# LemonATsu/UNet-PhaseGen

Measured on NVIDIA B200. Metric: audio_seconds_per_second_mag_to_phase_to_wave, higher is better.
Workload: dtype f16x3/f16x2/f16-fp32acc (two-product fp16 on d1,u2; single fp16 product = TF32 operand rounding on u1)

## Files before the change

unet-phasegen_b200/csrc/stft.cu:

```cuda
#include "common.cuh"
#include "stft_core.cuh"

namespace pg {
using namespace pgfft;

constexpr int kStftThreads = 256;

template <int NC> struct FrameCfg {
    static constexpr int TG = NC / 16;
    static constexpr int FC = kStftThreads / TG;
    static constexpr int NFFT = 2 * NC;
    static constexpr int HOP = NFFT / 4;
    static constexpr int PL = padded_len2(NC);
    static constexpr size_t smem_stft() { return sizeof(float2) * (Radix<NC, false>::TOTAL + NC + (size_t)FC * PL); }
    static constexpr int RING = FC + 3;
    static constexpr size_t smem_istft() { return sizeof(float2) * (Radix<NC, true>::TOTAL + NC + (size_t)RING * PL + NC ) + sizeof(float) * HOP; }
};

template <int TG> struct FrameSync {
    int slot;
    __device__ __forceinline__ void operator()() const {
        if (TG <= 32) __syncwarp();
        else asm volatile("bar.sync %0, %1;" ::"r"(slot + 1), "r"(TG) : "memory");
    }
};

__device__ __forceinline__ float fast_log1p_mag(float re, float im) {
    const float m2 = fmaf(re, re, im * im);
    float mag, l2;
    asm("sqrt.approx.ftz.f32 %0, %1;" : "=f"(mag) : "f"(m2));
    asm("lg2.approx.ftz.f32 %0, %1;" : "=f"(l2) : "f"(1.0f + mag));
    return l2 * 0.693147180559945f;
}

template <int NC, int FAST, bool RAGGED>
__global__ void __launch_bounds__(kStftThreads, 3)
stft_kernel(const float* __restrict__ wave, int N, int T, const float2* __restrict__ tw_g, int mode,
            float* __restrict__ out_a, float* __restrict__ out_b,
            uint16_t* __restrict__ op_hi, uint16_t* __restrict__ op_lo,
            long long op_batch_stride, int op_fmt, int frames_per_cta, const float* __restrict__ proj_mag,
            float std_mean, float std_inv, const int* __restrict__ clip_samples, const int* __restrict__ clip_frames) {
    using Cfg = FrameCfg<NC>;
    using R = Radix<NC, false>;
    extern __shared__ float2 smem2[];
    cpx* tabs = reinterpret_cast<cpx*>(smem2);
    cpx* win = tabs + R::TOTAL;
    cpx* bufs = win + NC;

    const int tid = threadIdx.x;
    const cpx* twc = reinterpret_cast<const cpx*>(tw_g);
    for (int e = tid; e < R::TOTAL; e += kStftThreads) tabs[e] = table_entry<NC, false>(twc, e);
    for (int m = tid; m < NC; m += kStftThreads)
        win[m] = {0.25f - 0.25f * tw_g[2 * m].x, 0.25f - 0.25f * tw_g[2 * m + 1].x};
    __syncthreads();

    const int b = blockIdx.y;
    const int n_b = RAGGED ? min(__ldg(clip_samples + b), N) : N;
    const int T_b = RAGGED ? min(__ldg(clip_frames + b), T) : T;
    const int N_b = RAGGED ? (T_b - 1) * Cfg::HOP : N;
    const int slot = tid / Cfg::TG, t = tid % Cfg::TG;
    cpx* s = bufs + slot * Cfg::PL;
    const FrameSync<Cfg::TG> sync{slot};
    const float* w = wave + (size_t)b * N;
    const bool aligned = (N & 1) == 0 && (reinterpret_cast<uintptr_t>(wave) & 7) == 0;
    const int f_begin = blockIdx.x * frames_per_cta;

    for (int f0 = f_begin; f0 < f_begin + frames_per_cta && f0 < T; f0 += Cfg::FC) {
        const int frame = f0 + slot;
        const bool live = frame < T;
        const int p0 = frame * Cfg::HOP - NC;
        cpx v[16];
        if (live && aligned && p0 >= 0 && p0 + Cfg::NFFT <= n_b) {
#pragma unroll
            for (int r = 0; r < 16; ++r) {
                const int m = t + r * Cfg::TG;
                const float2 xv = __ldg(reinterpret_cast<const float2*>(w + p0) + m);
                const cpx wv = win[m];
                v[r] = {xv.x * wv.x, xv.y * wv.y};
            }
        } else if (live && (!RAGGED || frame < T_b)) {
#pragma unroll
            for (int r = 0; r < 16; ++r) {
                const int m = t + r * Cfg::TG;
                int n0 = p0 + 2 * m, n1 = n0 + 1;
                if (n0 < 0) n0 = -n0;
                if (n0 >= N_b) n0 = 2 * (N_b - 1) - n0;
                if (n1 < 0) n1 = -n1;
                if (n1 >= N_b) n1 = 2 * (N_b - 1) - n1;
                const float x0 = (n0 >= 0 && n0 < n_b) ? __ldg(w + n0) : 0.f;
                const float x1 = (n1 >= 0 && n1 < n_b) ? __ldg(w + n1) : 0.f;
                const cpx wv = win[m];
                v[r] = {x0 * wv.x, x1 * wv.y};
            }
        } else {
#pragma unroll
            for (int r = 0; r < 16; ++r) v[r] = {0.f, 0.f};
        }
        fwd_phase0<NC>(s, t, v);
        sync();
        fwd_phase1<NC>(s, t, tabs, sync);
        sync();

        const size_t row = ((size_t)b * T + frame) * NC;
        const size_t orow = (size_t)b * op_batch_stride + (size_t)frame * NC;
        auto emit = [&](int bin, cpx x) {
            if (FAST) {
                const float a = fast_log1p_mag(x.x, x.y);
                uint16_t hi, lo;
                split16(a, FAST == 2 ? PG_FMT_F16 : PG_FMT_BF16, hi, lo);
                out_a[row + bin - 1] = a;
                op_hi[orow + bin - 1] = hi;
                op_lo[orow + bin - 1] = lo;
                return;
            }
            if (bin == NC) x.y = 0.f;
            float a, ph = 0.f;
            if (mode == PG_STFT_PROJECT) {
                const float m2 = fmaf(x.x, x.x, x.y * x.y);
                const float inv = m2 > 0.f ? rsqrtf(m2) : 0.f;
                const float g = __ldg(proj_mag + row + bin - 1);
                a = m2 > 0.f ? g * x.x * inv : g;
                ph = g * x.y * inv;
            } else if (mode == PG_STFT_LOGMAG || mode == PG_STFT_PAIRS) {
                if (mode == PG_STFT_PAIRS) {
                    x.x = (x.x - std_mean) * std_inv;
                    x.y = (x.y - std_mean) * std_inv;
                }
                a = fast_log1p_mag(x.x, x.y);
                if (out_b) ph = atan2f(x.y, x.x);
            } else {
                a = x.x; ph = x.y;
            }
            if (out_a) out_a[row + bin - 1] = a;
            if (out_b) out_b[row + bin - 1] = ph;
            if (op_hi) {
                uint16_t hi, lo;
                split16(a, op_fmt, hi, lo);
                op_hi[orow + bin - 1] = hi;
                if (op_lo) op_lo[orow + bin - 1] = lo;
            }
        };
        if (NC == 512) {
            if (live) fwd_fused_last_512(s, t, tabs, emit);
        } else {
            fwd_phase2_unfused<NC>(s, t, tabs, sync);
            sync();
            if (live) fwd_post_generic<NC>(s, t, tabs, emit);
        }
        sync();
    }
}

__device__ __forceinline__ cpx spec_value(float a, float p, int mode) {
    if (mode == PG_SPEC_CARTESIAN) return {a, p};
    float mag = a;
    if (mode == PG_SPEC_POLAR_LOG) mag = __expf(a) - 1.0f;
    return {mag * __cosf(p), mag * __sinf(p)};
}

template <int NC, bool FAST, bool RAGGED>
__global__ void __launch_bounds__(kStftThreads)
istft_kernel(const float* __restrict__ in_a, const float* __restrict__ in_b, int mode, int T,
             const float2* __restrict__ tw_g, float* __restrict__ wave,
             unsigned* __restrict__ peak_bits, int* __restrict__ nonfinite, int blocks_per_cta,
             const float2* __restrict__ b_ss, int b_ss_stride, const int* __restrict__ clip_frames,
             const int* __restrict__ clip_samples) {
    using Cfg = FrameCfg<NC>;
    using R = Radix<NC, true>;
    constexpr int FC = Cfg::FC, HOP = Cfg::HOP;
    extern __shared__ float2 smem2[];
    float* wss_full = reinterpret_cast<float*>(smem2);
    cpx* tabs = reinterpret_cast<cpx*>(wss_full + HOP);
    cpx* win = tabs + R::TOTAL;
    cpx* ring = win + NC;
    float2* ss_tab = reinterpret_cast<float2*>(ring + (size_t)Cfg::RING * Cfg::PL);

    const int tid = threadIdx.x;
    const cpx* twc = reinterpret_cast<const cpx*>(tw_g);
    for (int e = tid; e < R::TOTAL; e += kStftThreads) tabs[e] = table_entry<NC, true>(twc, e);
    for (int m = tid; m < NC; m += kStftThreads) win[m] = {0.5f - 0.5f * tw_g[2 * m].x, 0.5f - 0.5f * tw_g[2 * m + 1].x};
    for (int i = tid; i < HOP; i += kStftThreads) {
        float acc = 0.f;
#pragma unroll
        for (int q = 0; q < 4; ++q) { const float wn = 0.5f - 0.5f * tw_g[q * HOP + i].x; acc += wn * wn; }
        wss_full[i] = acc > 1.17549435e-38f ? 1.0f / acc : 1.0f;
    }
    const int b = blockIdx.y;
    const int T_b = RAGGED ? min(__ldg(clip_frames + b), T) : T;
    const int n_b = RAGGED ? __ldg(clip_samples + b) : 0;
    if (b_ss) for (int m = tid; m < NC; m += kStftThreads) ss_tab[m] = __ldg(b_ss + (size_t)b * b_ss_stride + m);
    __syncthreads();

    const int J0 = blockIdx.x * blocks_per_cta;
    const int J1 = min(J0 + blocks_per_cta, T - 1);
    const int F0 = J0 - 1;
    const int n_iter = (J1 - J0 + 3 + FC - 1) / FC;
    const int slot = tid / Cfg::TG, t = tid % Cfg::TG;
    const FrameSync<Cfg::TG> sync{slot};
    const float scale = 0.5f / NC;
    float* wv = wave + (size_t)b * (size_t)(T - 1) * HOP;
    float pk = 0.f;
    bool bad = false;

    float ra[16], rb[16];
    auto is_live = [&](int frame) { return frame >= 0 && frame < T_b && frame <= J1 + 1; };
    auto fetch = [&](int frame) {
        if (!is_live(frame)) return;
        const size_t row = ((size_t)b * T + frame) * NC;
#pragma unroll
        for (int j = 0; j < 16; ++j) {
            const size_t idx = row + inv_bin<NC>(t, j) - 1;
            ra[j] = __ldg(in_a + idx);
            rb[j] = (FAST || in_b) ? __ldg(in_b + idx) : 0.f;
        }
    };
    fetch(F0 + slot);

    for (int it = 0; it < n_iter; ++it) {
        const int F = F0 + it * FC;
        const int frame = F + slot;
        const bool live = is_live(frame);
        cpx* s = ring + (size_t)((frame - F0) % Cfg::RING) * Cfg::PL;
        if (live) {
            cpx x[16];
#pragma unroll
            for (int j = 0; j < 16; ++j) {
                float pb = rb[j];
                if (b_ss) { const float2 ss = ss_tab[inv_bin<NC>(t, j) - 1]; pb = fmaf(pb, ss.x, ss.y); }
                x[j] = spec_value(ra[j], pb, FAST ? (int)PG_SPEC_POLAR_LOG : mode);
            }
            if (NC == 512) inv_fused_first_512(s, t, tabs, scale, x);
            else inv_pre_generic<NC>(s, t, tabs, scale, x);
        }
        if (it + 1 < n_iter) fetch(frame + FC);
        sync();
        inv_passes<NC>(s, t, tabs, win, sync);
        __syncthreads();

        const int lo = max(J0, F - 2), hi = min(J1, F + FC - 2);
        for (int u = tid; u < (hi - lo) * (HOP / 4); u += kStftThreads) {
            const int jb = lo + u / (HOP / 4), i = (u % (HOP / 4)) * 4;
            float4 acc = make_float4(0.f, 0.f, 0.f, 0.f), wss;
            const bool interior = jb >= 1 && jb + 2 < T_b;
            if (interior) wss = *reinterpret_cast<const float4*>(wss_full + i);
            else wss = make_float4(0.f, 0.f, 0.f, 0.f);
#pragma unroll
            for (int q = 0; q < 4; ++q) {
                const int fr = jb - 1 + q;
                if (fr < 0 || fr >= T_b) continue;
                const cpx* fb = ring + (size_t)((fr - F0) % Cfg::RING) * Cfg::PL;
                const int m = ((3 - q) * HOP + i) >> 1;
                const cpx z0 = fb[pad2(m)], z1 = fb[pad2(m + 1)];
                acc.x += z0.x; acc.y += z0.y; acc.z += z1.x; acc.w += z1.y;
                if (!interior) {
                    const cpx w0 = win[m], w1 = win[m + 1];
                    wss.x += w0.x * w0.x; wss.y += w0.y * w0.y; wss.z += w1.x * w1.x; wss.w += w1.y * w1.y;
                }
            }
            if (!interior) {
                wss.x = wss.x > 1.17549435e-38f ? 1.0f / wss.x : 1.0f; wss.y = wss.y > 1.17549435e-38f ? 1.0f / wss.y : 1.0f;
                wss.z = wss.z > 1.17549435e-38f ? 1.0f / wss.z : 1.0f; wss.w = wss.w > 1.17549435e-38f ? 1.0f / wss.w : 1.0f;
            }
            float4 y;
            y.x = acc.x * wss.x; y.y = acc.y * wss.y; y.z = acc.z * wss.z; y.w = acc.w * wss.w;
            if (RAGGED && jb >= T_b - 1) y = make_float4(0.f, 0.f, 0.f, 0.f);
            const float mx = fmaxf(fmaxf(fabsf(y.x), fabsf(y.y)), fmaxf(fabsf(y.z), fabsf(y.w)));
            if (!(mx <= 3.402823466e+38f) || y.x != y.x || y.y != y.y || y.z != y.z || y.w != y.w) bad = true;
            pk = fmaxf(pk, mx);
            if (RAGGED) {
                const int n = jb * HOP + i;
                if (n >= n_b) y.x = 0.f;
                if (n + 1 >= n_b) y.y = 0.f;
                if (n + 2 >= n_b) y.z = 0.f;
                if (n + 3 >= n_b) y.w = 0.f;
            }
            *reinterpret_cast<float4*>(wv + (size_t)jb * HOP + i) = y;
        }
        __syncthreads();
    }
    if (peak_bits) {
#pragma unroll
        for (int o = 16; o; o >>= 1) pk = fmaxf(pk, __shfl_xor_sync(0xffffffffu, pk, o));
        if ((tid & 31) == 0 && pk > 0.f) atomicMax(peak_bits + b, __float_as_uint(pk));
    }
    if (nonfinite && bad) atomicOr(nonfinite + b, 1);
}

__global__ void peak_normalize_kernel(float* __restrict__ wave, const unsigned* __restrict__ peak_bits, int n) {
    const int b = blockIdx.y;
    float pk = __uint_as_float(peak_bits[b]);
    if (!(pk >= 1.17549435e-38f)) return;
    float inv = 1.0f / pk;
    float* w = wave + (size_t)b * n;
    if ((n & 3) == 0) {
        float4* w4 = reinterpret_cast<float4*>(w);
        for (int i = blockIdx.x * blockDim.x + threadIdx.x; i < n / 4; i += gridDim.x * blockDim.x) {
            float4 v = w4[i];
            v.x *= inv; v.y *= inv; v.z *= inv; v.w *= inv;
            w4[i] = v;
        }
    } else {
        for (int i = blockIdx.x * blockDim.x + threadIdx.x; i < n; i += gridDim.x * blockDim.x) w[i] = w[i] * inv;
    }
}

__global__ void __launch_bounds__(256)
stitch_kernel(const float* __restrict__ windows, int n_windows, int win, int step, int world, int per_rank,
              float* __restrict__ out, long long n_out, unsigned* __restrict__ peak_bits) {
    const int ov = win - step;
    const float inv_ov = ov > 0 ? 1.0f / (float)ov : 0.f;
    float pk = 0.f;
    for (long long n = (long long)blockIdx.x * blockDim.x + threadIdx.x; n < n_out; n += (long long)gridDim.x * blockDim.x) {
        long long i1 = n / step; if (i1 > n_windows - 1) i1 = n_windows - 1;
        float acc = 0.f;
#pragma unroll
        for (int q = 0; q < 2; ++q) {
            const long long i = i1 - q;
            if (i < 0) continue;
            const long long o = n - i * step;
            if (o >= win) continue;
            float g = 1.f;
            if (i > 0 && o < ov) g = 0.5f - 0.5f * cospif((float)o * inv_ov);
            else if (i < n_windows - 1 && o >= win - ov) g = 0.5f + 0.5f * cospif((float)(o - (win - ov)) * inv_ov);
            const size_t slot = (size_t)(i % world) * per_rank + (size_t)(i / world);
            acc = fmaf(__ldg(windows + slot * win + o), g, acc);
        }
        out[n] = acc;
        pk = fmaxf(pk, fabsf(acc));
    }
    if (peak_bits) {
#pragma unroll
        for (int o = 16; o; o >>= 1) pk = fmaxf(pk, __shfl_xor_sync(0xffffffffu, pk, o));
        if ((threadIdx.x & 31) == 0 && pk > 0.f) atomicMax(peak_bits, __float_as_uint(pk));
    }
}

template <int NC, bool RAGGED>
static auto stft_variant(bool fast, int fmt) {
    return !fast ? stft_kernel<NC, 0, RAGGED> : fmt == PG_FMT_F16 ? stft_kernel<NC, 2, RAGGED> : stft_kernel<NC, 1, RAGGED>;
}

template <int NC>
static int launch_stft(const float* wave, int B, int N, int T, const float* tw, int mode, float* a, float* bq,
                       uint16_t* hi, uint16_t* lo, long long bs, int fmt, cudaStream_t st, const float* proj_mag = nullptr,
                       float std_mean = 0.f, float std_inv = 1.f, const int* clip_samples = nullptr, const int* clip_frames = nullptr) {
    using Cfg = FrameCfg<NC>;
    const bool fast = mode == PG_STFT_LOGMAG && a && !bq && hi && lo;
    auto k = clip_samples ? stft_variant<NC, true>(fast, fmt) : stft_variant<NC, false>(fast, fmt);
    const size_t sm = Cfg::smem_stft();
    static bool configured_dev[kMaxDevices] = {};
    bool& configured = configured_dev[current_device_slot()];
    if (!configured) {
        for (int f = 0; f < 3; ++f)
            for (auto kv : {stft_variant<NC, false>(f > 0, f == 2 ? PG_FMT_F16 : PG_FMT_BF16),
                            stft_variant<NC, true>(f > 0, f == 2 ? PG_FMT_F16 : PG_FMT_BF16)})
                cudaFuncSetAttribute(kv, cudaFuncAttributeMaxDynamicSharedMemorySize, (int)sm);
        configured = true;
    }
    const int frames_per_cta = Cfg::FC * 4;
    dim3 grid((T + frames_per_cta - 1) / frames_per_cta, B);
    k<<<grid, kStftThreads, sm, st>>>(wave, N, T, reinterpret_cast<const float2*>(tw), mode, a, bq, hi, lo, bs, fmt, frames_per_cta, proj_mag,
                                      std_mean, std_inv, clip_samples, clip_frames);
    return check_launch("stft_kernel");
}

template <int NC>
static int launch_istft(const float* a, const float* bq, int mode, int B, int T, const float* tw, float* wave,
                        float* peak, int* nonfinite, cudaStream_t st, const float* b_ss, int b_ss_stride,
                        const int* clip_frames = nullptr, const int* clip_samples = nullptr) {
    using Cfg = FrameCfg<NC>;
    const bool fast = mode == PG_SPEC_POLAR_LOG && bq;
    auto k = clip_frames ? (fast ? istft_kernel<NC, true, true> : istft_kernel<NC, false, true>)
                         : (fast ? istft_kernel<NC, true, false> : istft_kernel<NC, false, false>);
    const size_t sm = Cfg::smem_istft();
    static bool configured_dev[kMaxDevices] = {};
    bool& configured = configured_dev[current_device_slot()];
    if (!configured) {
        for (auto kv : {istft_kernel<NC, true, false>, istft_kernel<NC, false, false>, istft_kernel<NC, true, true>, istft_kernel<NC, false, true>})
            cudaFuncSetAttribute(kv, cudaFuncAttributeMaxDynamicSharedMemorySize, (int)sm);
        configured = true;
    }
    const int blocks_per_cta = 11 * Cfg::FC - 3;
    dim3 grid((T - 1 + blocks_per_cta - 1) / blocks_per_cta, B);
    k<<<grid, kStftThreads, sm, st>>>(a, bq, mode, T, reinterpret_cast<const float2*>(tw), wave,
                                     reinterpret_cast<unsigned*>(peak), nonfinite, blocks_per_cta,
                                     reinterpret_cast<const float2*>(b_ss), b_ss_stride, clip_frames, clip_samples);
    return check_launch("istft_kernel");
}

}

extern "C" int pg_stft_num_frames(int n_samples, int hop) { return hop > 0 ? 1 + n_samples / hop : 0; }

static int stft_entry(const float* wave, int B, int N, int n_fft, int hop, const float* twiddle, int mode,
                      float* out_a, float* out_b, uint16_t* op_hi, uint16_t* op_lo,
                      int64_t op_batch_stride, int op_fmt, const int* cs, const int* cf, pg_stream stream) {
    PG_REQUIRE(wave && twiddle && B > 0 && N > 0, "pg_stft: null pointer or empty batch");
    PG_REQUIRE(hop * 4 == n_fft, "pg_stft: hop must be n_fft/4 (got n_fft=%d hop=%d)", n_fft, hop);
    PG_REQUIRE(N > n_fft / 2, "pg_stft: reflect padding needs more than n_fft/2 samples (N=%d)", N);
    PG_REQUIRE(mode == PG_STFT_LOGMAG || mode == PG_STFT_REIM, "pg_stft: bad mode %d", mode);
    PG_REQUIRE(B <= 65535, "pg_stft: batch too large for one launch");
    const int T = 1 + N / hop;
    cudaStream_t st = reinterpret_cast<cudaStream_t>(stream);
    switch (n_fft) {
        case 256:  return pg::launch_stft<128>(wave, B, N, T, twiddle, mode, out_a, out_b, op_hi, op_lo, op_batch_stride, op_fmt, st, nullptr, 0.f, 1.f, cs, cf);
        case 512:  return pg::launch_stft<256>(wave, B, N, T, twiddle, mode, out_a, out_b, op_hi, op_lo, op_batch_stride, op_fmt, st, nullptr, 0.f, 1.f, cs, cf);
        case 1024: return pg::launch_stft<512>(wave, B, N, T, twiddle, mode, out_a, out_b, op_hi, op_lo, op_batch_stride, op_fmt, st, nullptr, 0.f, 1.f, cs, cf);
        case 2048: return pg::launch_stft<1024>(wave, B, N, T, twiddle, mode, out_a, out_b, op_hi, op_lo, op_batch_stride, op_fmt, st, nullptr, 0.f, 1.f, cs, cf);
    }
    pg::set_error("pg_stft: n_fft must be 256, 512, 1024 or 2048 (got %d)", n_fft);
    return PG_ERR_UNSUPPORTED;
}

extern "C" int pg_stft(const float* wave, int B, int N, int n_fft, int hop, const float* twiddle, int mode,
                       float* out_a, float* out_b, uint16_t* op_hi, uint16_t* op_lo,
                       int64_t op_batch_stride, int op_fmt, pg_stream stream) {
    return stft_entry(wave, B, N, n_fft, hop, twiddle, mode, out_a, out_b, op_hi, op_lo, op_batch_stride, op_fmt, nullptr, nullptr, stream);
}

extern "C" int pg_stft_ragged(const float* wave, int B, int N, int n_fft, int hop, const float* twiddle, int mode,
                              float* out_a, float* out_b, uint16_t* op_hi, uint16_t* op_lo,
                              int64_t op_batch_stride, int op_fmt, const int* clip_samples, const int* clip_frames, pg_stream stream) {
    PG_REQUIRE(clip_samples && clip_frames, "pg_stft_ragged: null per-clip table");
    if (mode != PG_STFT_LOGMAG) {
        pg::set_error("pg_stft_ragged: only PG_STFT_LOGMAG takes per-clip lengths (got mode %d)", mode);
        return PG_ERR_UNSUPPORTED;
    }
    return stft_entry(wave, B, N, n_fft, hop, twiddle, mode, out_a, out_b, op_hi, op_lo, op_batch_stride, op_fmt, clip_samples, clip_frames, stream);
}

extern "C" int pg_stft_project(const float* wave, int B, int N, int n_fft, int hop, const float* twiddle, const float* mag,
                               float* out_re, float* out_im, pg_stream stream) {
    PG_REQUIRE(wave && twiddle && mag && out_re && out_im && B > 0 && N > 0, "pg_stft_project: null pointer or empty batch");
    PG_REQUIRE(hop * 4 == n_fft, "pg_stft_project: hop must be n_fft/4 (got n_fft=%d hop=%d)", n_fft, hop);
    PG_REQUIRE(N > n_fft / 2, "pg_stft_project: reflect padding needs more than n_fft/2 samples (N=%d)", N);
    PG_REQUIRE(B <= 65535, "pg_stft_project: batch too large for one launch");
    const int T = 1 + N / hop;
    cudaStream_t st = reinterpret_cast<cudaStream_t>(stream);
    switch (n_fft) {
        case 256:  return pg::launch_stft<128>(wave, B, N, T, twiddle, PG_STFT_PROJECT, out_re, out_im, nullptr, nullptr, 0, 0, st, mag);
        case 512:  return pg::launch_stft<256>(wave, B, N, T, twiddle, PG_STFT_PROJECT, out_re, out_im, nullptr, nullptr, 0, 0, st, mag);
        case 1024: return pg::launch_stft<512>(wave, B, N, T, twiddle, PG_STFT_PROJECT, out_re, out_im, nullptr, nullptr, 0, 0, st, mag);
        case 2048: return pg::launch_stft<1024>(wave, B, N, T, twiddle, PG_STFT_PROJECT, out_re, out_im, nullptr, nullptr, 0, 0, st, mag);
    }
    pg::set_error("pg_stft_project: n_fft must be 256, 512, 1024 or 2048 (got %d)", n_fft);
    return PG_ERR_UNSUPPORTED;
}

extern "C" int pg_stft_pairs(const float* wave, int B, int N, int n_fft, int hop, const float* twiddle, float mean, float std,
                             float* out_logmag, float* out_phase, pg_stream stream) {
    PG_REQUIRE(wave && twiddle && out_logmag && out_phase && B > 0 && N > 0, "pg_stft_pairs: null pointer or empty batch");
    PG_REQUIRE(hop * 4 == n_fft, "pg_stft_pairs: hop must be n_fft/4 (got n_fft=%d hop=%d)", n_fft, hop);
    PG_REQUIRE(N > n_fft / 2, "pg_stft_pairs: reflect padding needs more than n_fft/2 samples (N=%d)", N);
    PG_REQUIRE(std > 0.f && B <= 65535, "pg_stft_pairs: std must be positive and B <= 65535");
    const int T = 1 + N / hop;
    cudaStream_t st = reinterpret_cast<cudaStream_t>(stream);
    const float inv = 1.0f / std;
    switch (n_fft) {
        case 256:  return pg::launch_stft<128>(wave, B, N, T, twiddle, PG_STFT_PAIRS, out_logmag, out_phase, nullptr, nullptr, 0, 0, st, nullptr, mean, inv);
        case 512:  return pg::launch_stft<256>(wave, B, N, T, twiddle, PG_STFT_PAIRS, out_logmag, out_phase, nullptr, nullptr, 0, 0, st, nullptr, mean, inv);
        case 1024: return pg::launch_stft<512>(wave, B, N, T, twiddle, PG_STFT_PAIRS, out_logmag, out_phase, nullptr, nullptr, 0, 0, st, nullptr, mean, inv);
        case 2048: return pg::launch_stft<1024>(wave, B, N, T, twiddle, PG_STFT_PAIRS, out_logmag, out_phase, nullptr, nullptr, 0, 0, st, nullptr, mean, inv);
    }
    pg::set_error("pg_stft_pairs: n_fft must be 256, 512, 1024 or 2048 (got %d)", n_fft);
    return PG_ERR_UNSUPPORTED;
}

static int istft_entry(const float* in_a, const float* in_b, int mode, int B, int T, int n_fft, int hop,
                       const float* twiddle, float* wave, float* peak, int* nonfinite,
                       const float* b_scale_shift, int b_ss_per_clip, const int* cf, const int* cs, pg_stream stream) {
    PG_REQUIRE(in_a && twiddle && wave && B > 0 && T > 1, "pg_istft: null pointer or empty input");
    PG_REQUIRE(hop * 4 == n_fft, "pg_istft: hop must be n_fft/4 (got n_fft=%d hop=%d)", n_fft, hop);
    PG_REQUIRE(mode >= PG_SPEC_POLAR_LOG && mode <= PG_SPEC_POLAR_MAG, "pg_istft: bad mode %d", mode);
    PG_REQUIRE(in_b || mode != PG_SPEC_CARTESIAN, "pg_istft: second plane missing");
    PG_REQUIRE(B <= 65535, "pg_istft: batch too large for one launch");
    PG_REQUIRE(!b_scale_shift || in_b, "pg_istft: scale/shift given without a second plane");
    const int ss_stride = b_ss_per_clip ? n_fft / 2 : 0;
    cudaStream_t st = reinterpret_cast<cudaStream_t>(stream);
    if (peak) cudaMemsetAsync(peak, 0, sizeof(float) * B, st);
    if (nonfinite) cudaMemsetAsync(nonfinite, 0, sizeof(int) * B, st);
    switch (n_fft) {
        case 256:  return pg::launch_istft<128>(in_a, in_b, mode, B, T, twiddle, wave, peak, nonfinite, st, b_scale_shift, ss_stride, cf, cs);
        case 512:  return pg::launch_istft<256>(in_a, in_b, mode, B, T, twiddle, wave, peak, nonfinite, st, b_scale_shift, ss_stride, cf, cs);
        case 1024: return pg::launch_istft<512>(in_a, in_b, mode, B, T, twiddle, wave, peak, nonfinite, st, b_scale_shift, ss_stride, cf, cs);
        case 2048: return pg::launch_istft<1024>(in_a, in_b, mode, B, T, twiddle, wave, peak, nonfinite, st, b_scale_shift, ss_stride, cf, cs);
    }
    pg::set_error("pg_istft: n_fft must be 256, 512, 1024 or 2048 (got %d)", n_fft);
    return PG_ERR_UNSUPPORTED;
}

extern "C" int pg_istft(const float* in_a, const float* in_b, int mode, int B, int T, int n_fft, int hop,
                        const float* twiddle, float* wave, float* peak, int* nonfinite,
                        const float* b_scale_shift, int b_ss_per_clip, pg_stream stream) {
    return istft_entry(in_a, in_b, mode, B, T, n_fft, hop, twiddle, wave, peak, nonfinite, b_scale_shift, b_ss_per_clip, nullptr, nullptr, stream);
}

extern "C" int pg_istft_ragged(const float* in_a, const float* in_b, int mode, int B, int T, int n_fft, int hop,
                               const float* twiddle, float* wave, float* peak, int* nonfinite,
                               const float* b_scale_shift, int b_ss_per_clip, const int* clip_frames, const int* clip_samples,
                               pg_stream stream) {
    PG_REQUIRE(clip_frames && clip_samples, "pg_istft_ragged: null per-clip table");
    return istft_entry(in_a, in_b, mode, B, T, n_fft, hop, twiddle, wave, peak, nonfinite, b_scale_shift, b_ss_per_clip, clip_frames, clip_samples, stream);
}

extern "C" int pg_peak_normalize(float* wave, const float* peak, int B, int N, pg_stream stream) {
    PG_REQUIRE(wave && peak && B > 0 && N > 0 && B <= 65535, "pg_peak_normalize: bad arguments");
    dim3 grid((N + 1023) / 1024 < 64 ? (N + 1023) / 1024 : 64, B);
    pg::peak_normalize_kernel<<<grid, 256, 0, reinterpret_cast<cudaStream_t>(stream)>>>(
        wave, reinterpret_cast<const unsigned*>(peak), N);
    return pg::check_launch("peak_normalize_kernel");
}

extern "C" int pg_stitch(const float* windows, int n_windows, int win, int step, int world, int per_rank, float* out,
                         int64_t n_out, float* peak, pg_stream stream) {
    PG_REQUIRE(windows && out && n_windows > 0 && win > 0 && n_out > 0, "pg_stitch: bad arguments");
    PG_REQUIRE(step > 0 && step <= win && 2 * step >= win, "pg_stitch: step must lie in [win/2, win] (got win=%d step=%d)", win, step);
    PG_REQUIRE(world >= 1 && per_rank >= (n_windows + world - 1) / world, "pg_stitch: per_rank too small for %d windows on %d ranks", n_windows, world);
    PG_REQUIRE(n_out <= (int64_t)win + (int64_t)(n_windows - 1) * step, "pg_stitch: n_out exceeds the span of the windows");
    cudaStream_t st = reinterpret_cast<cudaStream_t>(stream);
    if (peak) cudaMemsetAsync(peak, 0, sizeof(float), st);
    long long blocks = (n_out + 255) / 256; if (blocks > 148 * 16) blocks = 148 * 16;
    pg::stitch_kernel<<<(int)blocks, 256, 0, st>>>(windows, n_windows, win, step, world, per_rank, out, n_out, reinterpret_cast<unsigned*>(peak));
    return pg::check_launch("stitch_kernel");
}
```

unet-phasegen_b200/phasegen/ops.py:

```python
import ctypes as C
import math

import torch

from . import _lib
from ._lib import (ActDst, ConvDesc, ConvEpilogue, PG_EPI_ACT, PG_EPI_NORM_ACT, PG_EPI_RAW, PG_CONV, PG_CONV_TRANSPOSE, PG_DT_BF16, PG_DT_BF16_SPLIT, PG_DT_F16,
                   PG_DT_F16_SPLIT, PG_DT_F32, PG_DT_NONE, PG_FMT_BF16, PG_FMT_F16, PG_PREC_BF16, PG_PREC_BF16X3,
                   PG_PREC_F16X2, PG_PREC_F16X3, PG_PREC_FP32_SIMT, PG_SPEC_CARTESIAN, PG_SPEC_POLAR_LOG,
                   PG_SPEC_POLAR_MAG, PG_STFT_LOGMAG, PG_STFT_REIM)

SUPPORTED_N_FFT = (256, 512, 1024, 2048)


def _stream(t=None):
    dev = t.device if isinstance(t, torch.Tensor) and t.is_cuda else None
    return C.c_void_p(torch.cuda.current_stream(dev).cuda_stream)


def _ptr(t):
    return C.c_void_p(t.data_ptr()) if t is not None else C.c_void_p(0)


def _fmt(t):
    if t is None or t.dtype == torch.bfloat16:
        return PG_FMT_BF16
    if t.dtype == torch.float16:
        return PG_FMT_F16
    raise RuntimeError(f"phasegen: operand planes must be bfloat16 or float16, got {t.dtype}")


def _need_cuda(t, name, dtype=torch.float32):
    if not isinstance(t, torch.Tensor) or not t.is_cuda:
        raise RuntimeError(f"phasegen: `{name}` must be a CUDA tensor (there is no CPU path)")
    if t.dtype != dtype:
        raise RuntimeError(f"phasegen: `{name}` must be {dtype}, got {t.dtype}")
    if t.device.index != torch.cuda.current_device():
        raise RuntimeError(f"phasegen: `{name}` lives on {t.device} but the current device is cuda:{torch.cuda.current_device()}; "
                           "wrap the call in `with torch.cuda.device(tensor.device):`")
    _lib.require_device(t.device.index)
    return t.contiguous()


_twiddles = {}


def twiddle(n_fft, device):
    key = (n_fft, str(device))
    if key not in _twiddles:
        m = torch.arange(n_fft, dtype=torch.float64)
        ang = -2.0 * math.pi * m / n_fft
        _twiddles[key] = torch.stack([torch.cos(ang), torch.sin(ang)], 1).float().contiguous().to(device)
    return _twiddles[key]


def check_stft_geometry(n_fft, hop):
    if n_fft not in SUPPORTED_N_FFT or hop * 4 != n_fft:
        raise RuntimeError(f"phasegen: n_fft must be one of {SUPPORTED_N_FFT} with hop = n_fft/4 "
                           f"(got n_fft={n_fft}, hop={hop})")


def _lengths(t, B, name):
    t = _need_cuda(t, name, torch.int32)
    if t.numel() != B:
        raise RuntimeError(f"phasegen: `{name}` must hold one entry per clip ({B}), got {t.numel()}")
    return t


def stft(wave, n_fft, hop, mode=PG_STFT_LOGMAG, want_second=True, operand=None, clip_samples=None, clip_frames=None):
    check_stft_geometry(n_fft, hop)
    wave = _need_cuda(wave, "wave")
    if wave.dim() != 2:
        raise RuntimeError("phasegen.stft: wave must be [B, N]")
    B, N = wave.shape
    T = 1 + N // hop
    Cb = n_fft // 2
    a = torch.empty(B, T, Cb, device=wave.device, dtype=torch.float32)
    b = torch.empty_like(a) if want_second else None
    hi, lo, bs = operand if operand is not None else (None, None, 0)
    if clip_samples is not None or clip_frames is not None:
        _lib.call("pg_stft_ragged", _ptr(wave), B, N, n_fft, hop, _ptr(twiddle(n_fft, wave.device)), mode,
                  _ptr(a), _ptr(b), _ptr(hi), _ptr(lo), bs, _fmt(hi), _ptr(_lengths(clip_samples, B, "clip_samples")),
                  _ptr(_lengths(clip_frames, B, "clip_frames")), _stream())
        return a, b
    _lib.call("pg_stft", _ptr(wave), B, N, n_fft, hop, _ptr(twiddle(n_fft, wave.device)), mode,
              _ptr(a), _ptr(b), _ptr(hi), _ptr(lo), bs, _fmt(hi), _stream())
    return a, b


def stft_project(wave, mag, n_fft, hop, out=None):
    check_stft_geometry(n_fft, hop)
    wave = _need_cuda(wave, "wave")
    mag = _need_cuda(mag, "mag")
    B, N = wave.shape
    T = 1 + N // hop
    if tuple(mag.shape) != (B, T, n_fft // 2):
        raise RuntimeError(f"phasegen.stft_project: mag must be [{B}, {T}, {n_fft // 2}], got {tuple(mag.shape)}")
    re, im = out if out is not None else (torch.empty_like(mag), torch.empty_like(mag))
    _lib.call("pg_stft_project", _ptr(wave), B, N, n_fft, hop, _ptr(twiddle(n_fft, wave.device)), _ptr(mag),
              _ptr(re), _ptr(im), _stream())
    return re, im


def stft_pairs(wave, n_fft, hop, mean=0.0, std=1.0):
    check_stft_geometry(n_fft, hop)
    wave = _need_cuda(wave, "wave")
    B, N = wave.shape
    T = 1 + N // hop
    lm = torch.empty(B, T, n_fft // 2, device=wave.device, dtype=torch.float32)
    ph = torch.empty_like(lm)
    _lib.call("pg_stft_pairs", _ptr(wave), B, N, n_fft, hop, _ptr(twiddle(n_fft, wave.device)), float(mean), float(std),
              _ptr(lm), _ptr(ph), _stream())
    return lm, ph


def istft(a, b, mode, n_fft, hop, normalize=True, check_finite=True, out=None, b_scale_shift=None, bad_out=None,
          clip_frames=None, clip_samples=None):
    check_stft_geometry(n_fft, hop)
    a = _need_cuda(a, "a")
    b = _need_cuda(b, "b") if b is not None else None
    B, T, Cb = a.shape
    if Cb != n_fft // 2 or (b is not None and b.shape != a.shape):
        raise RuntimeError("phasegen.istft: inputs must be [B, T, n_fft/2] and of equal shape")
    n = (T - 1) * hop
    if out is not None and (tuple(out.shape) != (B, n) or out.dtype != torch.float32 or not out.is_cuda or not out.is_contiguous()):
        raise RuntimeError(f"phasegen.istft: `out` must be a contiguous CUDA float32 [{B}, {n}] tensor")
    wave = out if out is not None else torch.empty(B, n, device=a.device, dtype=torch.float32)
    peak = torch.empty(B, device=a.device, dtype=torch.float32)
    bad = bad_out if bad_out is not None else torch.empty(B, device=a.device, dtype=torch.int32)
    per_clip = 0
    if b_scale_shift is not None:
        b_scale_shift = _need_cuda(b_scale_shift, "b_scale_shift")
        if b_scale_shift.numel() not in (2 * Cb, 2 * Cb * B):
            raise RuntimeError("phasegen.istft: b_scale_shift must hold (scale, shift) per bin, for all clips or per clip")
        per_clip = int(b_scale_shift.numel() == 2 * Cb * B and B > 1)
    if clip_frames is not None or clip_samples is not None:
        _lib.call("pg_istft_ragged", _ptr(a), _ptr(b), mode, B, T, n_fft, hop, _ptr(twiddle(n_fft, a.device)),
                  _ptr(wave), _ptr(peak), _ptr(bad), _ptr(b_scale_shift), per_clip,
                  _ptr(_lengths(clip_frames, B, "clip_frames")), _ptr(_lengths(clip_samples, B, "clip_samples")), _stream())
    else:
        _lib.call("pg_istft", _ptr(a), _ptr(b), mode, B, T, n_fft, hop, _ptr(twiddle(n_fft, a.device)),
                  _ptr(wave), _ptr(peak), _ptr(bad), _ptr(b_scale_shift), per_clip, _stream())
    if normalize:
        _lib.call("pg_peak_normalize", _ptr(wave), _ptr(peak), B, n, _stream())
    if check_finite and bool(bad.any().item()):
        raise ValueError("Audio buffer is not finite everywhere")
    return wave, peak


def transpose(src, dst=None, dst_hi=None, dst_lo=None, dst_batch_stride=None, dst_ld=None, range_flag=None):
    src = _need_cuda(src, "src")
    B, R, S = src.shape
    if dst is None and dst_hi is None:
        dst = torch.empty(B, S, R, device=src.device, dtype=torch.float32)
    ld = R if dst_ld is None else dst_ld
    bs = S * ld if dst_batch_stride is None else dst_batch_stride
    _lib.call("pg_transpose", _ptr(src), B, R, S, R * S, _ptr(dst), _ptr(dst_hi), _ptr(dst_lo), bs, ld, _fmt(dst_hi), _ptr(range_flag), _stream())
    return dst


def conv_desc(kind, B, C_in, C_out, L_in, k, stride, pad, in_rows, in_ld, precision, L_out=None,
              out_rows=None, out_ld=None, taps_per_group=0, base_offset_mode=0, max_ctas=0, max_clips_per_tile=0, weights_mn_major=0, cta_pair=0,
              whole_clip=0):
    if L_out is None:
        L_out = (L_in - 1) * stride - 2 * pad + k if kind == PG_CONV_TRANSPOSE else (L_in + 2 * pad - k) // stride + 1
    return ConvDesc(kind, B, C_in, C_out, L_in, L_out, k, stride, pad, in_rows, in_ld,
                    L_out if out_rows is None else out_rows, C_out if out_ld is None else out_ld,
                    precision, taps_per_group, base_offset_mode, max_ctas, max_clips_per_tile, weights_mn_major, cta_pair, whole_clip)


def pack_weight(w, kind, want_tc=True, want_simt=False, plane_dtype=torch.bfloat16, want_lo=True):
    w = _need_cuda(w.detach(), "weight")
    if kind == PG_CONV_TRANSPOSE:
        C_in, C_out, k = w.shape
    else:
        C_out, C_in, k = w.shape
    hi = lo = simt = None
    if want_tc:
        hi = torch.empty(k, C_out, C_in, device=w.device, dtype=plane_dtype)
        lo = torch.empty_like(hi) if want_lo else None
    if want_simt:
        simt = torch.empty(k, C_in, C_out, device=w.device, dtype=torch.float32)
    _lib.call("pg_pack_weight", _ptr(w), kind, C_in, C_out, k, _ptr(hi), _ptr(lo), _ptr(simt), _fmt(hi), _stream())
    return hi, lo, simt


def conv_tc(desc, x_hi, x_lo, w_hi, w_lo, y, stats, epilogue=None, out_rows=None):
    if out_rows is not None:
        _lib.call("pg_conv_tc_ragged", C.byref(desc), _ptr(x_hi), _ptr(x_lo), _ptr(w_hi), _ptr(w_lo), _ptr(y), _ptr(stats),
                  C.byref(epilogue) if epilogue is not None else None, _ptr(_lengths(out_rows, desc.B, "out_rows")), _stream())
        return
    _lib.call("pg_conv_tc", C.byref(desc), _ptr(x_hi), _ptr(x_lo), _ptr(w_hi), _ptr(w_lo), _ptr(y), _ptr(stats),
              C.byref(epilogue) if epilogue is not None else None, _stream())


_NO_DST = ActDst(None, None, 0, 0, 0, PG_DT_NONE, 1.0, None)


def conv_epilogue(mode, dst0, dst1=None, gamma=None, beta=None, eps=1e-5, scale_shift=None):
    return ConvEpilogue(mode, gamma.data_ptr() if gamma is not None else None, beta.data_ptr() if beta is not None else None,
                        float(eps), dst0, dst1 if dst1 is not None else _NO_DST,
                        scale_shift.data_ptr() if scale_shift is not None else None)


def conv_epilogue_supported(desc, mode):
    r = _lib.load().pg_conv_epilogue_supported(C.byref(desc), mode)
    if r < 0:
        raise RuntimeError(f"pg_conv_epilogue_supported failed ({r}): {_lib.last_error()}")
    return bool(r)


def conv_stat_parts(desc):
    p = _lib.load().pg_conv_stat_parts(C.byref(desc))
    if p <= 0:
        raise RuntimeError(f"pg_conv_stat_parts failed ({p}): {_lib.last_error()}")
    return p


_PLAN_KEYS = ("n_tile", "n_ntiles", "nb", "strip_rows", "pair", "merged", "mgroups", "acc_stages", "n_chunks", "n_cotiles",
              "OS", "IS", "taps0", "taps1", "groups0", "groups1", "whole_clip")


def conv_plan(desc, whole_clip=None):
    d = ConvDesc.from_buffer_copy(desc)
    if whole_clip is not None:
        d.tc_whole_clip = int(whole_clip)
    out = (C.c_int * 17)()
    if _lib.load().pg_conv_tc_plan(C.byref(d), out, 17) != 0:
        return None
    pl = dict(zip(_PLAN_KEYS, out))
    slabs = pl["n_cotiles"] // 2 if pl["pair"] else pl["n_cotiles"]
    parts = 1 if pl["whole_clip"] else pl["OS"] * pl["n_ntiles"]
    pl["tiles"] = slabs * parts * -(-d.B // pl["nb"])
    pl["units"] = 74 if pl["pair"] else 148
    return pl


def conv_simt(desc, x, w_simt, y):
    _lib.call("pg_conv_simt", C.byref(desc), _ptr(x), _ptr(w_simt), _ptr(y), _stream())


def channel_stats(y, B, L, Cn, rows, ld, stats):
    _lib.call("pg_channel_stats", _ptr(y), B, L, Cn, rows, ld, _ptr(stats), _stream())


def bn_finalize(stats, B, P, Cn, per_clip, gamma, beta, eps, scale_shift, mean_var=None):
    _lib.call("pg_bn_finalize", _ptr(stats), B, P, Cn, int(per_clip), _ptr(gamma), _ptr(beta), eps,
              _ptr(scale_shift), _ptr(mean_var), _stream())


def act_dst(hi, lo, batch_stride, ld, ch_off, dtype, slope, range_flag=None):
    return ActDst(hi.data_ptr() if hi is not None else None, lo.data_ptr() if lo is not None else None,
                  batch_stride, ld, ch_off, dtype, slope, range_flag.data_ptr() if range_flag is not None else None)


def bn_running_update(mean_var, running_mean, running_var, momentum, unbias):
    Cn = running_mean.numel()
    for t, name in ((mean_var, "mean_var"), (running_mean, "running_mean"), (running_var, "running_var")):
        _need_cuda(t, name)
        if t.dtype != torch.float32 or not t.is_contiguous():
            raise RuntimeError(f"phasegen.bn_running_update: {name} must be a contiguous float32 CUDA tensor")
    if mean_var.numel() < 2 * Cn or running_var.numel() != Cn:
        raise RuntimeError("phasegen.bn_running_update: shapes do not match")
    _lib.call("pg_bn_running_update", _ptr(mean_var), _ptr(running_mean), _ptr(running_var), Cn, float(momentum), float(unbias), _stream())


def bn_from_running(running_mean, running_var, gamma, beta, eps, scale_shift, mean_var=None):
    G, Cn = scale_shift.shape[0], scale_shift.shape[1]
    _lib.call("pg_bn_from_running", _ptr(running_mean), _ptr(running_var), _ptr(gamma), _ptr(beta), float(eps), Cn, G,
              _ptr(scale_shift), _ptr(mean_var), _stream())


def bn_act(y, B, L, Cn, rows, ld, scale_shift, per_clip, dst0, dst1=None, clip_rows=None):
    if clip_rows is not None:
        _lib.call("pg_bn_act_ragged", _ptr(y), B, L, Cn, rows, ld, _ptr(scale_shift), int(per_clip),
                  C.byref(dst0), C.byref(dst1) if dst1 is not None else None, _ptr(_lengths(clip_rows, B, "clip_rows")), _stream())
        return
    _lib.call("pg_bn_act", _ptr(y), B, L, Cn, rows, ld, _ptr(scale_shift), int(per_clip),
              C.byref(dst0), C.byref(dst1) if dst1 is not None else None, _stream())


def grad_src(g, ld, ch_off, slope):
    return _lib.GradSrc(g.data_ptr(), ld, ch_off, slope)


def phase_loss(out_cl, logmag_cl, phase_cl, d_out, partial, loss3, mag_weight=0.2):
    B, T, C2 = out_cl.shape
    _lib.call("pg_phase_loss", _ptr(out_cl), _ptr(logmag_cl), _ptr(phase_cl), B * T, C2 // 2, mag_weight,
              _ptr(d_out), _ptr(partial), partial.shape[0], _ptr(loss3), _stream(), n_kernels=2)


def bn_bwd(z, B, L, Cn, scale_shift, mean_var, eps, g0, g1, partial, coef, dgamma, dbeta, dz_hi, dz_lo, dz_rows, dz_dtype):
    n_chunks = partial.shape[0] if partial is not None else 0
    _lib.call("pg_bn_bwd", _ptr(z), B, L, Cn, _ptr(scale_shift), _ptr(mean_var), eps, C.byref(g0),
              C.byref(g1) if g1 is not None else None, _ptr(partial), n_chunks, _ptr(coef), _ptr(dgamma), _ptr(dbeta),
              _ptr(dz_hi), _ptr(dz_lo), dz_rows, dz_dtype, _stream(), n_kernels=3 if scale_shift is not None else 1)


def wgrad_tc(desc, x_hi, x_lo, g_hi, g_lo, g_rows, dw_packed):
    dt = PG_DT_BF16 if dw_packed.dtype == torch.bfloat16 else PG_DT_F32
    _lib.call("pg_wgrad_tc", C.byref(desc), _ptr(x_hi), _ptr(x_lo), _ptr(g_hi), _ptr(g_lo), g_rows, _ptr(dw_packed), dt, _stream())


def wgrad_simt(desc, x, g, g_rows, dw_packed):
    _lib.call("pg_wgrad_simt", C.byref(desc), _ptr(x), _ptr(g), g_rows, _ptr(dw_packed), _stream())


def unpack_grad(packed, kind, out):
    k, C_out, C_in = packed.shape
    _lib.call("pg_unpack_grad", _ptr(packed), kind, C_in, C_out, k, _ptr(out), _stream())


def adam_step(p, g, m, v, lr, beta1, beta2, eps, step, grad_scale=1.0, w_hi=None, w_lo=None):
    gdt = PG_DT_BF16 if g.dtype == torch.bfloat16 else PG_DT_F32
    _lib.call("pg_adam_step", _ptr(p), _ptr(g), gdt, _ptr(m), _ptr(v), p.numel(), lr, beta1, beta2, eps, step, grad_scale,
              _ptr(w_hi), _ptr(w_lo), _stream())


def cast_split(src, hi, lo=None, range_flag=None):
    _lib.call("pg_cast_split", _ptr(src), src.numel(), _ptr(hi), _ptr(lo), _fmt(hi), _ptr(range_flag), _stream())


def packed_view(weight, kind):
    w = weight.detach()
    v = w.permute(2, 1, 0) if kind == PG_CONV_TRANSPOSE else w.permute(2, 0, 1)
    return v if v.is_contiguous() else None


def to_packed_storage(weight, kind):
    w = weight.detach()
    packed = (w.permute(2, 1, 0) if kind == PG_CONV_TRANSPOSE else w.permute(2, 0, 1)).contiguous()
    return packed.permute(2, 1, 0) if kind == PG_CONV_TRANSPOSE else packed.permute(1, 2, 0)
```

Measured before the change: 45880.

## Stage iSTFT input rows via cp.async into ring slots and size grid by occupancy

The iSTFT kernel now copies each frame's magnitude and phase rows into its shared-memory ring slot with coalesced 16-byte cp.async, and issues L2 bulk prefetches for the next frame. This replaces the per-thread scattered __ldg register prefetch. The launcher also picks the number of CTAs per clip from SM count and occupancy, replacing the fixed frames-per-CTA constant, and sets a launch-bounds minimum-blocks hint. In exchange the kernel adds extra syncs, removes the register-level overlap of the next frame's load with compute, and requires 16-byte-aligned inputs, cloning them in Python when they are not.

```diff
diff --git a/unet-phasegen_b200/csrc/stft.cu b/unet-phasegen_b200/csrc/stft.cu
--- a/unet-phasegen_b200/csrc/stft.cu
+++ b/unet-phasegen_b200/csrc/stft.cu
@@ -15,6 +15,7 @@
     static constexpr size_t smem_stft() { return sizeof(float2) * (Radix<NC, false>::TOTAL + NC + (size_t)FC * PL); }
     static constexpr int RING = FC + 3;
     static constexpr size_t smem_istft() { return sizeof(float2) * (Radix<NC, true>::TOTAL + NC + (size_t)RING * PL + NC ) + sizeof(float) * HOP; }
+    static constexpr int ISTFT_CTAS = (int)(233472 / (smem_istft() + 1024)) < 3 ? (int)(233472 / (smem_istft() + 1024)) : 3;
 };
 
 template <int TG> struct FrameSync {
@@ -151,6 +152,15 @@
     }
 }
 
+__device__ __forceinline__ void cp_async16(float* dst, const float* src) {
+    const unsigned d = (unsigned)__cvta_generic_to_shared(dst);
+    asm volatile("cp.async.cg.shared.global [%0], [%1], 16;" ::"r"(d), "l"(src) : "memory");
+}
+__device__ __forceinline__ void cp_async_wait_all() { asm volatile("cp.async.wait_all;" ::: "memory"); }
+__device__ __forceinline__ void prefetch_l2(const float* src, unsigned bytes) {
+    asm volatile("cp.async.bulk.prefetch.L2.global [%0], %1;" ::"l"(src), "r"(bytes) : "memory");
+}
+
 __device__ __forceinline__ cpx spec_value(float a, float p, int mode) {
     if (mode == PG_SPEC_CARTESIAN) return {a, p};
     float mag = a;
@@ -159,7 +169,7 @@
 }
 
 template <int NC, bool FAST, bool RAGGED>
-__global__ void __launch_bounds__(kStftThreads)
+__global__ void __launch_bounds__(kStftThreads, FrameCfg<NC>::ISTFT_CTAS)
 istft_kernel(const float* __restrict__ in_a, const float* __restrict__ in_b, int mode, int T,
              const float2* __restrict__ tw_g, float* __restrict__ wave,
              unsigned* __restrict__ peak_bits, int* __restrict__ nonfinite, int blocks_per_cta,
@@ -168,12 +178,13 @@
     using Cfg = FrameCfg<NC>;
     using R = Radix<NC, true>;
     constexpr int FC = Cfg::FC, HOP = Cfg::HOP;
+    static_assert((HOP * 4) % 16 == 0 && (Cfg::PL * 8) % 16 == 0 && Cfg::PL >= NC, "ring slots: 16-byte aligned, hold both rows");
     extern __shared__ float2 smem2[];
     float* wss_full = reinterpret_cast<float*>(smem2);
-    cpx* tabs = reinterpret_cast<cpx*>(wss_full + HOP);
+    cpx* ring = reinterpret_cast<cpx*>(wss_full + HOP);
+    cpx* tabs = ring + (size_t)Cfg::RING * Cfg::PL;
     cpx* win = tabs + R::TOTAL;
-    cpx* ring = win + NC;
-    float2* ss_tab = reinterpret_cast<float2*>(ring + (size_t)Cfg::RING * Cfg::PL);
+    float2* ss_tab = reinterpret_cast<float2*>(win + NC);
 
     const int tid = threadIdx.x;
     const cpx* twc = reinterpret_cast<const cpx*>(tw_g);
@@ -202,25 +213,43 @@
     float pk = 0.f;
     bool bad = false;
 
-    float ra[16], rb[16];
+    const bool has_b = FAST || in_b;
     auto is_live = [&](int frame) { return frame >= 0 && frame < T_b && frame <= J1 + 1; };
-    auto fetch = [&](int frame) {
-        if (!is_live(frame)) return;
-        const size_t row = ((size_t)b * T + frame) * NC;
-#pragma unroll
-        for (int j = 0; j < 16; ++j) {
-            const size_t idx = row + inv_bin<NC>(t, j) - 1;
-            ra[j] = __ldg(in_a + idx);
-            rb[j] = (FAST || in_b) ? __ldg(in_b + idx) : 0.f;
-        }
-    };
-    fetch(F0 + slot);
+    auto row_of = [&](int frame) { return ((size_t)b * T + frame) * NC; };
+    if (t == 0 && is_live(F0 + slot)) {
+        prefetch_l2(in_a + row_of(F0 + slot), NC * 4);
+        if (has_b) prefetch_l2(in_b + row_of(F0 + slot), NC * 4);
+    }
 
     for (int it = 0; it < n_iter; ++it) {
         const int F = F0 + it * FC;
         const int frame = F + slot;
         const bool live = is_live(frame);
         cpx* s = ring + (size_t)((frame - F0) % Cfg::RING) * Cfg::PL;
+        float* sa = reinterpret_cast<float*>(s);
+        if (live) {
+            const size_t row = row_of(frame);
+#pragma unroll
+            for (int c = 0; c < NC / (4 * Cfg::TG); ++c) {
+                const int e = 4 * (t + c * Cfg::TG);
+                cp_async16(sa + e, in_a + row + e);
+                if (has_b) cp_async16(sa + NC + e, in_b + row + e);
+            }
+            if (t == 0 && it + 1 < n_iter && is_live(frame + FC)) {
+                prefetch_l2(in_a + row_of(frame + FC), NC * 4);
+                if (has_b) prefetch_l2(in_b + row_of(frame + FC), NC * 4);
+            }
+        }
+        cp_async_wait_all();
+        sync();
+        float ra[16], rb[16];
+#pragma unroll
+        for (int j = 0; j < 16; ++j) {
+            const int bin = inv_bin<NC>(t, j) - 1;
+            ra[j] = sa[bin];
+            rb[j] = has_b ? sa[NC + bin] : 0.f;
+        }
+        sync();
         if (live) {
             cpx x[16];
 #pragma unroll
@@ -232,7 +261,6 @@
             if (NC == 512) inv_fused_first_512(s, t, tabs, scale, x);
             else inv_pre_generic<NC>(s, t, tabs, scale, x);
         }
-        if (it + 1 < n_iter) fetch(frame + FC);
         sync();
         inv_passes<NC>(s, t, tabs, win, sync);
         __syncthreads();
@@ -373,15 +401,28 @@
     auto k = clip_frames ? (fast ? istft_kernel<NC, true, true> : istft_kernel<NC, false, true>)
                          : (fast ? istft_kernel<NC, true, false> : istft_kernel<NC, false, false>);
     const size_t sm = Cfg::smem_istft();
-    static bool configured_dev[kMaxDevices] = {};
-    bool& configured = configured_dev[current_device_slot()];
-    if (!configured) {
+    static int slots_dev[kMaxDevices] = {};
+    int& slots = slots_dev[current_device_slot()];
+    if (!slots) {
         for (auto kv : {istft_kernel<NC, true, false>, istft_kernel<NC, false, false>, istft_kernel<NC, true, true>, istft_kernel<NC, false, true>})
             cudaFuncSetAttribute(kv, cudaFuncAttributeMaxDynamicSharedMemorySize, (int)sm);
-        configured = true;
-    }
-    const int blocks_per_cta = 11 * Cfg::FC - 3;
-    dim3 grid((T - 1 + blocks_per_cta - 1) / blocks_per_cta, B);
+        int dev = 0, sms = 0, per_sm = 0;
+        cudaGetDevice(&dev);
+        cudaDeviceGetAttribute(&sms, cudaDevAttrMultiProcessorCount, dev);
+        cudaOccupancyMaxActiveBlocksPerMultiprocessor(&per_sm, istft_kernel<NC, true, false>, kStftThreads, sm);
+        slots = sms * per_sm > 0 ? sms * per_sm : 1;
+    }
+    int best_c = 1;
+    long long best_cost = -1;
+    for (int c = 1; c <= T - 1 && c <= 64; ++c) {
+        const int run = (T - 1 + c - 1) / c;
+        if (c > 1 && (T - 1 + run - 1) / run < c) continue;
+        const long long waves = ((long long)B * c + slots - 1) / slots;
+        const long long cost = waves * ((run + 3 + Cfg::FC - 1) / Cfg::FC + 1);
+        if (best_cost < 0 || cost < best_cost) { best_cost = cost; best_c = c; }
+    }
+    const int blocks_per_cta = (T - 1 + best_c - 1) / best_c;
+    dim3 grid(best_c, B);
     k<<<grid, kStftThreads, sm, st>>>(a, bq, mode, T, reinterpret_cast<const float2*>(tw), wave,
                                      reinterpret_cast<unsigned*>(peak), nonfinite, blocks_per_cta,
                                      reinterpret_cast<const float2*>(b_ss), b_ss_stride, clip_frames, clip_samples);
@@ -475,6 +516,8 @@
     PG_REQUIRE(in_b || mode != PG_SPEC_CARTESIAN, "pg_istft: second plane missing");
     PG_REQUIRE(B <= 65535, "pg_istft: batch too large for one launch");
     PG_REQUIRE(!b_scale_shift || in_b, "pg_istft: scale/shift given without a second plane");
+    PG_REQUIRE((reinterpret_cast<uintptr_t>(in_a) & 15) == 0 && (reinterpret_cast<uintptr_t>(in_b) & 15) == 0,
+               "pg_istft: input planes must be 16-byte aligned");
     const int ss_stride = b_ss_per_clip ? n_fft / 2 : 0;
     cudaStream_t st = reinterpret_cast<cudaStream_t>(stream);
     if (peak) cudaMemsetAsync(peak, 0, sizeof(float) * B, st);
diff --git a/unet-phasegen_b200/phasegen/ops.py b/unet-phasegen_b200/phasegen/ops.py
--- a/unet-phasegen_b200/phasegen/ops.py
+++ b/unet-phasegen_b200/phasegen/ops.py
@@ -121,6 +121,8 @@
     B, T, Cb = a.shape
     if Cb != n_fft // 2 or (b is not None and b.shape != a.shape):
         raise RuntimeError("phasegen.istft: inputs must be [B, T, n_fft/2] and of equal shape")
+    a = a if a.data_ptr() % 16 == 0 else a.clone()
+    b = b if b is None or b.data_ptr() % 16 == 0 else b.clone()
     n = (T - 1) * hop
     if out is not None and (tuple(out.shape) != (B, n) or out.dtype != torch.float32 or not out.is_cuda or not out.is_contiguous()):
         raise RuntimeError(f"phasegen.istft: `out` must be a contiguous CUDA float32 [{B}, {n}] tensor")
```

Result: no change. 45850, median of 6 (-0.1%).
